# cxjyxxme/deep-online-video-stabilization

Hardware: AMD Instinct MI355X
Metric: stabilized frames/sec (720p, before_ch=31) (higher is better)
Workload: dtype f32 (bf16x3 split MFMA, f32 accumulate); 1 GPU; BASELINE.json configs[1]: v2_93 net, 1280x720, 1 stream(s)/GPU, batch=1 per stream, 13-ch stack from a 32-deep ring (lags 1,2,4,8,16,32; --before-ch 31 ignored as in the reference), ResNet-v2-50 regressor + 4x4 multi-grid warp + feedback; one independent stream set per GPU (replicas only); height=720, width=1280, streams_per_gpu=1, refine=1, operand_mode=4, launches_per_frame=64, hip_graph=True

## Files before the change

deep-online-video-stabilization_amd/csrc/conv.h:

```cpp
#pragma once
#include "common.h"

struct ConvArgs {
    const float* x;
    const float* w;
    float* y;
    const float* bias;
    const float* in_scale;
    const float* in_shift;
    const float* residual;
    const float* out_scale;
    const float* out_shift;
    const float* out_floor;
    float* partial;
    int N, H, W, Cin, Ho, Wo, Cout, KH, KW, stride, pad;
    int up;
    int res_H, res_W, res_stride;
    int relu_out;
    int x_ld, res_ld;
    int M, K;
    int splitk, steps_per_split;
    int cin_real;
    unsigned div_hw_mul, div_hw_shift, div_w_mul, div_w_shift;
    int rowrun;
    int in_scale_expected;
    int xcd_swizzle;
};

size_t conv_plan(ConvArgs& a);
struct Prof;
int conv_launch(const ConvArgs& a, hipStream_t st, Prof* prof = nullptr, int bf16_operands = 0, const float* w_img = nullptr,
                bool lowk_ring = false);

enum ConvFamily {
    CONV_IGEMM,
    CONV_RING,
    CONV_RING_KG,
    CONV_RING_PRO,
    CONV_PACKED,
    CONV_PACKED_KG2,
    CONV_ASTAT
};
struct ConvRoute {
    int family;
    int tile, bk, nbuf;
    int mode;
    int operand;
    int kg, pro;
    int reduce;
    int prof_kind;
    int astat_bm;
};
ConvRoute conv_route(const ConvArgs& a, int operand_mode, bool has_image, bool bound, bool lowk_ring = false );
const char* conv_prof_kind_name(int kind);
size_t conv_weight_image_floats(int Cout, int K);
int launch_weight_split_image(const float* w, int Cout, int K, float* img, hipStream_t st);
struct WeightImageTable { long w_off[64], img_off[64], tprefix[65]; int Cout[64], K[64]; int n; };
void weight_image_table_add(WeightImageTable& t, long w_off, long img_off, int Cout, int K);
int launch_weight_split_images(const float* w_base, float* img_base, const WeightImageTable& t, hipStream_t st);
int conv_reduce_launches(const ConvArgs& a, int operand_mode = 0);

struct ConvPair { int m_tower, x_tower_floats ; long dx, dy, dres, dscale; };
bool conv_pair_supported(const ConvArgs& a);
int conv_launch_pair(const ConvArgs& a, const ConvPair& pr, hipStream_t st, Prof* prof = nullptr,
                     const float* w_img = nullptr );

bool conv_b2b_supported(const ConvArgs& c2, const ConvArgs& c3);
int conv_b2b_launch(const ConvArgs& c2, const ConvArgs& c3, hipStream_t st, Prof* prof = nullptr);

static inline void sn_fastdiv_make(unsigned d, unsigned& mul, unsigned& shift) {
    unsigned l = 0;
    while ((1ull << l) < d) ++l;
    mul = (unsigned)((((1ull << l) - d) << 32) / d + 1);
    shift = l;
}
#ifdef __HIPCC__
__device__ __forceinline__ int sn_fastdiv(int n, unsigned mul, unsigned shift) {
    return (int)((__umulhi(mul, (unsigned)n) + (unsigned)n) >> shift);
}
#endif
```

deep-online-video-stabilization_amd/csrc/conv.hip:

```cpp
#include "conv.h"
#include "prof.h"
#include <climits>
#include <cstdio>
#include <cstdlib>
#include <algorithm>
#include <string>
#include <vector>

#include "conv_kernel.h"
#include "conv_ring_kernel.h"
#include "conv_astat_kernel.h"
#include "conv_b2b_kernel.h"

template <int PAIR>
__device__ __forceinline__ void conv_splitk_reduce_body(const ConvArgs& p, const ConvPair& pr) {
    const size_t q = (size_t)blockIdx.x * 256 + threadIdx.x;
    const int c4n = p.Cout / 4;
    if (q >= (size_t)p.M * c4n) return;
    const int m = (int)(q / c4n);
    const int n = (int)(q - (size_t)m * c4n) * 4;
    const bool t1 = PAIR && m >= pr.m_tower;
    const size_t slab = (size_t)p.M * p.Cout;
    const float* src = p.partial + (size_t)m * p.Cout + n;
    float4 s = *reinterpret_cast<const float4*>(src);
    for (int z = 1; z < p.splitk; ++z) {
        const float4 t = *reinterpret_cast<const float4*>(src + z * slab);
        s.x += t.x; s.y += t.y; s.z += t.z; s.w += t.w;
    }
    if (p.bias != nullptr) {
        const float4 b = *reinterpret_cast<const float4*>(p.bias + n);
        s.x += b.x; s.y += b.y; s.z += b.z; s.w += b.w;
    }
    if (p.residual != nullptr) {
        size_t ri;
        if (p.res_stride == 1 && p.res_H == p.Ho && p.res_W == p.Wo) {
            ri = (size_t)m * p.res_ld + n;
        } else {
            const int img = sn_fastdiv(m, p.div_hw_mul, p.div_hw_shift);
            const int rr = m - img * (p.Ho * p.Wo);
            const int oy = sn_fastdiv(rr, p.div_w_mul, p.div_w_shift), ox = rr - oy * p.Wo;
            ri = (((size_t)img * p.res_H + oy * p.res_stride) * p.res_W + ox * p.res_stride) * p.res_ld + n;
        }
        const float4 t = *reinterpret_cast<const float4*>(p.residual + (t1 ? pr.dres : 0) + ri);
        s.x += t.x; s.y += t.y; s.z += t.z; s.w += t.w;
// ... 16 lines not shown
}
__global__ __launch_bounds__(256) void conv_splitk_reduce_pair_kernel(const ConvArgs p, const ConvPair pr) {
    conv_splitk_reduce_body<1>(p, pr);
}

enum TileId { T128x128 = 0, T128x64 = 1, T64x64 = 2 };

static void tile_dims(int t, int& bm, int& bn) {
    bm = (t == T64x64) ? 64 : 128;
    bn = (t == T128x128) ? 128 : 64;
}

static int env_int(const char* name, int dflt) {
    const char* v = getenv(name);
    return v ? atoi(v) : dflt;
}

struct ConvSwitches {
    int tile = env_int("STABNET_CONV_TILE", -1), splitk = env_int("STABNET_CONV_SPLITK", -1);
    int bk16 = env_int("STABNET_CONV_BK16", 0);
    int nbuf = env_int("STABNET_CONV_NBUF", 0);
    int tuning_table = env_int("STABNET_CONV_TUNING_TABLE", 1);
    int split_below = env_int("STABNET_CONV_SPLIT_BELOW", 400), split_target = env_int("STABNET_CONV_SPLIT_TARGET", 448);
    int xcd = env_int("STABNET_CONV_XCD", 1);
    int ring = env_int("STABNET_CONV_RING", 1), ring_wgs_per_cu = env_int("STABNET_CONV_RING_WGS_PER_CU", 3);
    int lowk_igemm = env_int("STABNET_CONV_LOWK_IGEMM", 1);
    int ring_pro = env_int("STABNET_CONV_RING_PRO", 1);
    int kgroups = env_int("STABNET_CONV_KGROUPS", 1), kgroups_pro = env_int("STABNET_CONV_KGROUPS_PRO", 1);
    int packed_kg2 = env_int("STABNET_CONV_PACKED_KG2", 1), packed_kg3 = env_int("STABNET_CONV_PACKED_KG3", 1);
    int packed_pro = env_int("STABNET_CONV_PACKED_PRO", 1);
    int packed_wgs_per_cu = env_int("STABNET_CONV_PACKED_WGS_PER_CU", 2);
    int astat = env_int("STABNET_CONV_ASTAT", 1), astat_min_m = env_int("STABNET_CONV_ASTAT_MIN_M", 0);
    int astat_min_cout = env_int("STABNET_CONV_ASTAT_MIN_COUT", 256);
    int b2b = env_int("STABNET_CONV_B2B", 1), b2b_wgs_per_cu = env_int("STABNET_CONV_B2B_WGS_PER_CU", 2);
};
static const ConvSwitches& sw() {
    static const ConvSwitches s;
    return s;
}

static int g_force_tile = -2, g_force_split = -1;
static int force_tile() { return g_force_tile == -2 ? sw().tile : g_force_tile; }
static int force_split() { return g_force_tile == -2 ? sw().splitk : g_force_split; }

static int conv_bk(const ConvArgs& a) { return (a.rowrun || (a.Cin % 32 == 0 && !sw().bk16)) ? 32 : 16; }
static int conv_total_steps(const ConvArgs& a) {
    if (a.rowrun) return a.KH * cdiv(a.KW * a.Cin, 32);
    return a.KH * a.KW * (a.Cin / conv_bk(a));
}

struct TuneEntry { int M, Cout, K, KH, ring, splitk; };
#include "conv_tuning_table.h"
#include "conv_tuning_table_packed.h"
static int g_tuning_profile = 0;
static std::vector<TuneEntry> g_tuning_runtime;

static int tuning_lookup(int M, int Cout, int K, int KH, int ring) {
    for (const TuneEntry& e : g_tuning_runtime)
        if (e.M == M && e.Cout == Cout && e.K == K && e.KH == KH && e.ring == ring) return e.splitk;
    if (sw().tuning_table && g_tuning_profile == 1)
        for (const TuneEntry& e : g_tuning_packed)
            if (e.M == M && e.Cout == Cout && e.K == K && e.KH == KH && e.ring == ring) return e.splitk;
    if (sw().tuning_table)
        for (const TuneEntry& e : g_tuning_builtin)
            if (e.M == M && e.Cout == Cout && e.K == K && e.KH == KH && e.ring == ring) return e.splitk;
    return 0;
// ... 43 lines not shown
    const int nbuf = sw().nbuf;
    bf16_out = (bm == 64 && bn == 64 && bk == 32) ? operand : 0;
    const bool one_stage = nbuf == 1 || (nbuf == 0 && mode == 0 && bm == 64 && bn == 64 && a.M >= 32768);
    nbuf_out = (bf16_out != 1 && one_stage) ? 1 : 2;
}

static bool ring_eligible(const ConvArgs& a, int tile, bool has_prologue, bool lowk_ring = false) {
    if (a.rowrun) return true;
    if (!lowk_ring && sw().lowk_igemm && a.KH == 1 && a.KW == 1 && a.Cin == 64 && a.x_ld == a.Cin && a.out_floor == nullptr) return false;
    return sw().ring && tile == T64x64 && !has_prologue && a.up == 1 && a.Cin % 32 == 0 && !sw().bk16;
}

static bool ring_pro_vectors_ok(const ConvArgs& a) {
    if (a.in_scale == nullptr || a.in_shift == nullptr) return true;
    const long d = (long)(a.in_shift - a.in_scale);
    return d >= 0 && d < (1L << 30);
}
static bool ring_pro_geometry(const ConvArgs& a, int operand, bool has_prologue) {
    return sw().ring_pro && sw().ring && operand != 1 && !sw().bk16 && has_prologue && a.KH == 1 && a.KW == 1 && a.stride == 1 && a.pad == 0 &&
           a.up == 1 && a.Cin % 32 == 0 && !a.rowrun && a.x_ld == a.Cin;
}
static bool ring_pro_eligible(const ConvArgs& a, int operand) {
    return ring_pro_geometry(a, operand, a.in_scale != nullptr) && a.out_scale == nullptr && a.out_floor == nullptr && ring_pro_vectors_ok(a);
}

static int conv_kgroups(const ConvArgs& a, int operand, bool ring, bool has_prologue) {
    if (!sw().kgroups || a.splitk < 2 || operand == 1) return 1;
    if (a.steps_per_split * a.splitk != conv_total_steps(a)) return 1;
    if (ring && a.splitk == 3 && !a.rowrun) return 3;
    if (sw().kgroups_pro && !ring && a.splitk == 2 && ring_pro_geometry(a, operand, has_prologue) && ring_pro_vectors_ok(a)) return 2;
    return 1;
}

static int route_prof_kind(const ConvRoute& r) {
    switch (r.family) {
        case CONV_IGEMM:
            return PK_KERNEL_CONV_BASE + r.mode * 6 + r.tile * 2 + (r.bk == 32 ? 1 : 0) + (r.nbuf == 1 ? 18 : 0) + 36 * r.operand;
        case CONV_PACKED: return PK_KERNEL_CONV_PACKED + (r.pro ? 3 : r.mode);
        case CONV_PACKED_KG2: return PK_KERNEL_CONV_PACKED + (r.pro ? 6 : 4 + r.mode);
        case CONV_ASTAT: return PK_KERNEL_CONV_ASTAT;
        default: break;
    }
    const int split = r.operand >= 2 ? PK_KERNEL_CONV_SPLIT + 8 * (r.operand - 2) : 0;
    if (r.family == CONV_RING) return split ? split + r.mode : PK_KERNEL_CONV_RING + r.mode + (r.operand ? 3 : 0);
    if (r.family == CONV_RING_PRO) return split ? split + 5 : PK_KERNEL_CONV_KG + 2;
    if (r.kg == 2) return split ? split + 6 : PK_KERNEL_CONV_KG + 3;
    return split ? split + 3 + r.mode : PK_KERNEL_CONV_KG + r.mode;
}

ConvRoute conv_route(const ConvArgs& a, int operand_mode, bool has_image, bool bound, bool lowk_ring) {
    const ConvSwitches& s = sw();
    const bool image = operand_mode == 4 && has_image;
    const int op = operand_mode == 4 ? 0 : operand_mode;
    int splitk_unused = 1;
    const int t = pick_tile(a, splitk_unused);
    const bool t64 = t == T64x64, bk32 = conv_bk(a) == 32;
    const bool has_pro = bound ? a.in_scale != nullptr : a.in_scale_expected != 0;
    const bool ring = ring_eligible(a, t, has_pro, lowk_ring && image);
    const bool slabs = !bound || a.splitk == 1 || a.partial != nullptr;
    int kg = t64 ? conv_kgroups(a, op, ring, has_pro) : 1;
    if (image && s.packed_kg3 && ring && kg == 3 && a.K % 32 == 0 && slabs) kg = 1;
    const bool pro = kg == 1 && !ring && t64 && bk32 && (bound ? ring_pro_eligible(a, op) : ring_pro_geometry(a, op, has_pro));
    const bool packed_pro = image && s.packed_pro && !ring && t64 && bk32 && ring_pro_geometry(a, op, has_pro) &&
                            (!bound || a.out_floor == nullptr)  && ring_pro_vectors_ok(a) && slabs;
    if (packed_pro) kg = 1;
    const bool packed = (image && ring && kg == 1 && a.K % 32 == 0) || packed_pro;
    const bool packed_kg2 = packed && s.packed_kg2 && a.splitk == 2 && !a.rowrun && a.steps_per_split * 2 == conv_total_steps(a);
    if (packed_kg2) kg = 2;
    const int astat_min_m = s.astat_min_m > 0 ? s.astat_min_m : ((long)a.Cout * a.K >= 128 * 1024 ? 2048 : 8192);
    const bool astat = packed && !packed_pro && !packed_kg2 && kg == 1 && a.splitk == 1 && s.astat && !lowk_ring && !a.rowrun &&
                       a.KH == 1 && a.KW == 1 && a.stride == 1 && a.pad == 0 && a.up == 1 && a.K <= 256 && a.Cout >= s.astat_min_cout &&
                       a.M >= astat_min_m;

    ConvRoute r{};
    r.tile = t;
    r.bk = bk32 ? 32 : 16;
    r.mode = (a.up > 1 || a.rowrun) ? 2 : (a.pad == 0 ? 0 : 1);
    r.operand = op;
    r.kg = kg;
    r.reduce = (a.splitk > 1 && kg == 1) ? 1 : 0;
    if (astat) {
        r.family = CONV_ASTAT;
        r.operand = 4;
        r.astat_bm = 32;
    } else if (packed) {
        r.family = packed_kg2 ? CONV_PACKED_KG2 : CONV_PACKED;
        r.operand = 4;
        r.pro = packed_pro ? 1 : 0;
    } else if (pro) {
        r.family = CONV_RING_PRO;
        r.pro = 1;
    } else if (kg > 1) {
        r.family = CONV_RING_KG;
        r.pro = kg == 2 ? 1 : 0;
    } else if (ring) {
        r.family = CONV_RING;
    } else {
        int bm, bn;
        tile_dims(t, bm, bn);
        r.family = CONV_IGEMM;
        igemm_variant(a, bm, bn, r.bk, r.mode, op, r.nbuf, r.operand);
    }
    r.prof_kind = route_prof_kind(r);
    return r;
}

int conv_reduce_launches(const ConvArgs& a, int operand_mode) {
    return a.splitk < 2 ? 0 : conv_route(a, operand_mode, operand_mode == 4, false).reduce;
}

const char* conv_prof_kind_name(int kind) {
    static const std::vector<std::string> names = [] {
        std::vector<std::string> v(PK_KERNEL_CONV_BASE + 144);
        char buf[96];
        auto ring = [&](int family, int mode, int operand, int kg, int pro) {
            ConvRoute r{};
            r.family = family; r.mode = mode; r.operand = operand; r.kg = kg; r.pro = pro;
            snprintf(buf, sizeof(buf), "conv_ring_f32_kernel<%d, %d, %d, %d>", mode, operand, kg, pro);
            v[route_prof_kind(r)] = buf;
        };
        for (int operand = 0; operand < 4; ++operand) {
            for (int mode = 0; mode < 3; ++mode) ring(CONV_RING, mode, operand, 1, 0);
            if (operand == 1) continue;
            ring(CONV_RING_KG, 0, operand, 3, 0); ring(CONV_RING_KG, 1, operand, 3, 0);
            ring(CONV_RING_PRO, 0, operand, 1, 1); ring(CONV_RING_KG, 0, operand, 2, 1);
        }
        for (int mode = 0; mode < 3; ++mode) ring(CONV_PACKED, mode, 4, 1, 0);
        ring(CONV_PACKED, 0, 4, 1, 1);
        ring(CONV_PACKED_KG2, 0, 4, 2, 0); ring(CONV_PACKED_KG2, 1, 4, 2, 0); ring(CONV_PACKED_KG2, 0, 4, 2, 1);
        {
            ConvRoute r{};
            r.family = CONV_ASTAT; r.astat_bm = 32;
            snprintf(buf, sizeof(buf), "conv_astat_f32_kernel<%d>", r.astat_bm);
            v[route_prof_kind(r)] = buf;
        }
        for (int i = 0; i < 144; ++i) {
            ConvRoute r{};
            r.family = CONV_IGEMM;
            r.operand = i / 36; r.nbuf = 2 - i / 18 % 2; r.mode = i / 6 % 3; r.tile = i / 2 % 3; r.bk = (i & 1) ? 32 : 16;
            int bm, bn;
            tile_dims(r.tile, bm, bn);
            snprintf(buf, sizeof(buf), "conv_igemm_f32_kernel<%d, %d, %d, %d, %d, %d, %d, %d>", bm, bn, r.bk, bm / 2, bn / 2, r.mode, r.nbuf, r.operand);
            v[route_prof_kind(r)] = buf;
        }
        for (int i = 0; i < 4; ++i) {
            snprintf(buf, sizeof(buf), "conv_igemm_f32_pair_kernel<64, 64, %d, 32, 32, %d>", (i & 1) ? 32 : 16, i / 2);
            v[PK_KERNEL_CONV_PAIR + i] = buf;
        }
        v[PK_KERNEL_CONV_B2B] = "conv_b2b_f32_kernel<2>";
        v[PK_KERNEL_CONV_B2B + 1] = "conv_b2b_f32_kernel<4>";
        return v;
    }();
    return (kind >= 0 && kind < (int)names.size() && !names[kind].empty()) ? names[kind].c_str() : nullptr;
}

template <int BM, int BN, int BK, int WM, int WN, int MODE, int NBUF, int BF16 = 0>
static int launch_one_nb(const ConvArgs& a, hipStream_t st) {
    constexpr size_t lds_op = NBUF * (size_t)(BM + BN) * (BK + 4) * sizeof(float);
    constexpr size_t lds_epi = 4 * (size_t)SN_EPI_WAVE_BYTES;
    constexpr size_t lds = lds_op > lds_epi ? lds_op : lds_epi;
    static bool configured = false;
    auto kern = conv_igemm_f32_kernel<BM, BN, BK, WM, WN, MODE, NBUF, BF16>;
    if (!configured) {
        if (lds > 64 * 1024) {
            hipError_t e = hipFuncSetAttribute(reinterpret_cast<const void*>(kern),
                                               hipFuncAttributeMaxDynamicSharedMemorySize, (int)lds);
            if (e != hipSuccess) {
                stabnet_set_error("conv: hipFuncSetAttribute(%zu B LDS) failed: %s", lds, hipGetErrorString(e));
// ... 76 lines not shown
static int launch_ring_route(const ConvRoute& r, const ConvArgs& a, hipStream_t st) {
    int cus = 0;
    if (const int rc = device_cus(cus)) return rc;
    const int per_cu = r.kg > 1 ? 1 : (r.operand == 4 ? sw().packed_wgs_per_cu : sw().ring_wgs_per_cu);
    const long ntiles = (long)cdiv(a.M, 64) * cdiv(a.Cout, 64) * (r.kg > 1 ? 1 : a.splitk);
    const int grid = (int)std::min<long>(ntiles, (long)per_cu * usable_cus(cus));
    bool ok = false;
    switch (r.operand) {
        case 0: ok = launch_ring_operand<0>(r, a, grid, st); break;
        case 1: ok = launch_ring_operand<1>(r, a, grid, st); break;
        case 2: ok = launch_ring_operand<2>(r, a, grid, st); break;
        case 3: ok = launch_ring_operand<3>(r, a, grid, st); break;
        case 4: ok = launch_ring_operand<4>(r, a, grid, st); break;
        default: break;
    }
    SN_REQUIRE(ok, "conv: no conv_ring_f32_kernel<%d, %d, %d, %d>", r.mode, r.operand, r.kg, r.pro);
    SN_LAUNCH_CHECK("conv_ring_f32_kernel");
    return STABNET_OK;
}

static int launch_astat(const ConvRoute& r, const ConvArgs& a, hipStream_t st) {
    int cus = 0;
    if (const int rc = device_cus(cus)) return rc;
    const int bm = r.astat_bm;
    SN_REQUIRE(bm == 32 && a.K % 32 == 0 && (size_t)bm * a.K * 6 <= (size_t)SN_ASTAT_A_BYTES && a.splitk == 1,
               "conv: the A-stationary kernel takes BM %d x K %d without a K split only if the planes fit %d bytes", bm, a.K, SN_ASTAT_A_BYTES);
    const int mtiles = cdiv(a.M, bm), nblk = 2 * cdiv(a.Cout, 64);
    int groups = (int)std::min<long>(cdiv(nblk, 4), std::max<long>(1, 2L * usable_cus(cus) / mtiles));
    groups = cdiv(nblk, 4 * cdiv(cdiv(nblk, groups), 4));
    const dim3 grid(mtiles, groups);
    conv_astat_f32_kernel<32><<<grid, 256, 0, st>>>(a);
    SN_LAUNCH_CHECK("conv_astat_f32_kernel");
    return STABNET_OK;
}

size_t conv_weight_image_floats(int Cout, int K) { return (size_t)cdiv(Cout, 64) * (size_t)(K / 32) * 3072; }

__device__ __forceinline__ unsigned weight_split_head(float& x0, float& x1) {
    const float top = __builtin_bit_cast(float, 0x7F7F0000u), fmax = __builtin_bit_cast(float, 0x7F7FFFFFu);
    const float h0 = (fabsf(x0) > top && fabsf(x0) <= fmax) ? copysignf(top, x0) : x0;
    const float h1 = (fabsf(x1) > top && fabsf(x1) <= fmax) ? copysignf(top, x1) : x1;
    const unsigned p = sn_pack_bf16(h0, h1);
    x0 = sn_sub_f32(x0, __builtin_bit_cast(float, p << 16));
    x1 = sn_sub_f32(x1, __builtin_bit_cast(float, p & 0xffff0000u));
    return p;
}
__device__ __forceinline__ SnSplit3 weight_split3(const f32x4 x) {
    float a = x.x, b = x.y, c = x.z, d = x.w;
    typedef unsigned u32x2 __attribute__((ext_vector_type(2)));
    u32x2 h, m, l;
    h.x = weight_split_head(a, b); h.y = weight_split_head(c, d);
    m.x = sn_split_level(a, b); m.y = sn_split_level(c, d);
    l.x = sn_pack_bf16(a, b); l.y = sn_pack_bf16(c, d);
    SnSplit3 s;
    s.h = __builtin_bit_cast(sn_bf16x4, h); s.m = __builtin_bit_cast(sn_bf16x4, m); s.l = __builtin_bit_cast(sn_bf16x4, l);
    return s;
}

__device__ __forceinline__ void weight_split_image_thread(const float* __restrict__ w, int Cout, int K, uint4* __restrict__ img, long i) {
    const int steps = K / 32;
    const int lane = (int)(i & 63), j = (int)((i >> 6) & 1), wn = (int)((i >> 7) & 1);
    const long ts = i >> 8;
    const int ks = (int)(ts % steps), nt = (int)(ts / steps);
    const int n = nt * 64 + wn * 32 + (lane & 31), g = lane >> 5;
    f32x4 lo = {0.f, 0.f, 0.f, 0.f}, hi = lo;
    if (n < Cout) {
// ... 39 lines not shown

int launch_weight_split_image(const float* w, int Cout, int K, float* img, hipStream_t st) {
    SN_REQUIRE(w && img && Cout > 0 && K > 0 && K % 32 == 0, "weight image: K=%d must be a multiple of 32", K);
    const long total = (long)cdiv(Cout, 64) * (K / 32) * 256;
    weight_split_image_kernel<<<cdiv(total, 256), 256, 0, st>>>(w, Cout, K, reinterpret_cast<uint4*>(img));
    SN_LAUNCH_CHECK("weight_split_image_kernel");
    return STABNET_OK;
}

int conv_launch(const ConvArgs& a, hipStream_t st, Prof* prof, int bf16_operands, const float* w_img, bool lowk_ring) {
    SN_REQUIRE(a.rowrun || a.Cin % 16 == 0, "conv: Cin=%d must be a multiple of 16 (pad the channels)", a.Cin);
    SN_REQUIRE(!a.rowrun || (a.in_scale == nullptr && a.up == 1 && a.KH <= 8 && cdiv(a.KW * a.Cin, 32) <= 4),
               "conv: row-run operand needs no prologue, KH <= 8 and KW*Cin <= 128");
    SN_REQUIRE(a.Cout % 4 == 0, "conv: Cout=%d must be a multiple of 4", a.Cout);
    SN_REQUIRE(a.splitk >= 1 && a.steps_per_split >= 1 && a.div_hw_mul != 0, "conv: conv_plan() not called");
    SN_REQUIRE(a.splitk == 1 || a.partial != nullptr, "conv: split-K needs a workspace");
    const ConvRoute r = conv_route(a, bf16_operands, w_img != nullptr, true, lowk_ring);
    SN_REQUIRE(r.family != CONV_IGEMM || a.x_ld == a.Cin, "conv: a strided input (x_ld %d != Cin %d) needs the ring kernel", a.x_ld, a.Cin);
    const bool rec = prof != nullptr && prof->begin(st);
    int rc;
    switch (r.family) {
        case CONV_IGEMM: rc = launch_igemm(r, a, st); break;
        case CONV_PACKED:
        case CONV_PACKED_KG2: {
            ConvArgs b = a;
            b.w = w_img;
            rc = launch_ring_route(r, b, st);
            break;
        }
        case CONV_ASTAT: {
            ConvArgs b = a;
            b.w = w_img;
            rc = launch_astat(r, b, st);
            break;
        }
        default: rc = launch_ring_route(r, a, st); break;
    }
    if (rec) prof->end(st, r.prof_kind, 2.0 * a.M * (double)(a.KH * a.KW * (a.cin_real ? a.cin_real : a.Cin)) * a.Cout,
                       4.0 * ((double)a.N * a.H * a.W * a.Cin + (double)a.K * a.Cout + (double)a.M * a.Cout * (r.reduce ? a.splitk : 1) +
                              ((a.residual != nullptr && !r.reduce) ? (double)a.M * a.Cout : 0.0)),
                       a.M, a.Cout, a.K, a.splitk);
    if (rc) return rc;
    if (r.reduce) {
        const size_t q = (size_t)a.M * (a.Cout / 4);
        const bool rec2 = prof != nullptr && prof->begin(st);
        conv_splitk_reduce_kernel<<<cdiv((long)q, 256), 256, 0, st>>>(a);
        if (rec2) prof->end(st, PK_KERNEL_SPLITK_REDUCE, 0.0, 4.0 * (double)a.M * a.Cout * (a.splitk + 1 + (a.residual != nullptr ? 1 : 0)));
        SN_LAUNCH_CHECK("conv_splitk_reduce_kernel");
    }
    return STABNET_OK;
}

bool conv_pair_supported(const ConvArgs& a) {
    int splitk_unused = 1;
    const int t = pick_tile(a, splitk_unused);
    const bool pro = a.in_scale != nullptr || a.in_scale_expected;
    return t == T64x64 && !ring_eligible(a, t, pro) && a.up == 1 && !a.rowrun && (a.x_ld == 0 || a.x_ld == a.Cin);
}

template <int BK, int MODE>
static int launch_pair_one(const ConvArgs& a, const ConvPair& pr, hipStream_t st) {
    constexpr size_t lds = 2 * (size_t)(64 + 64) * (BK + 4) * sizeof(float);
    static_assert(lds >= 4 * (size_t)SN_EPI_WAVE_BYTES && lds <= 64 * 1024, "LDS of the 64x64 tile");
    dim3 grid(cdiv(a.M, 64), cdiv(a.Cout, 64), a.splitk);
    conv_igemm_f32_pair_kernel<64, 64, BK, 32, 32, MODE><<<grid, 256, lds, st>>>(a, pr);
    SN_LAUNCH_CHECK("conv_igemm_f32_pair_kernel");
// ... 148 lines not shown
                          int Cout, int KH, int KW, int stride, int pad, int relu_out, void* workspace,
                          size_t workspace_bytes, void* stream);

int stabnet_conv2d_fwd(const float* x, const float* w_ohwi, const float* bias, const float* in_scale,
                       const float* in_shift, const float* residual, int res_H, int res_W, int res_stride, float* y,
                       int N, int H, int W, int Cin, int Cout, int KH, int KW, int stride, int pad, int relu_out,
                       void* workspace, size_t workspace_bytes, void* stream) {
    return stabnet_conv2d_fwd_ex(x, w_ohwi, bias, in_scale, in_shift, residual, res_H, res_W, res_stride, nullptr, nullptr,
                                 y, N, H, W, Cin, Cout, KH, KW, stride, pad, relu_out, workspace, workspace_bytes, stream);
}

int stabnet_conv2d_fwd_ex(const float* x, const float* w_ohwi, const float* bias, const float* in_scale,
                          const float* in_shift, const float* residual, int res_H, int res_W, int res_stride,
                          const float* out_scale, const float* out_shift, float* y, int N, int H, int W, int Cin,
                          int Cout, int KH, int KW, int stride, int pad, int relu_out, void* workspace,
                          size_t workspace_bytes, void* stream) {
    SN_REQUIRE(x && w_ohwi && y, "conv2d_fwd: null pointer");
    SN_REQUIRE((out_scale == nullptr) == (out_shift == nullptr), "conv2d_fwd: out_scale and out_shift go together");
    ConvArgs a;
    int rc = fill_args(a, x, w_ohwi, bias, in_scale, in_shift, residual, res_H, res_W, res_stride, y, N, H, W, Cin, Cout,
                       KH, KW, stride, pad, relu_out);
    if (rc) return rc;
    const size_t need = conv_plan(a);
    if (need > workspace_bytes || (need > 0 && workspace == nullptr)) {
        stabnet_set_error("conv2d_fwd: workspace %zu B < %zu B needed", workspace_bytes, need);
        return STABNET_ERR_WORKSPACE;
    }
    a.partial = static_cast<float*>(workspace);
    a.out_scale = out_scale;
    a.out_shift = out_shift;
    return conv_launch(a, (hipStream_t)stream);
}

size_t stabnet_conv_weight_image_floats(int Cout, int KH, int KW, int Cin) {
    const int K = KH * KW * Cin;
    return (Cout > 0 && K > 0 && K % 32 == 0) ? conv_weight_image_floats(Cout, K) : 0;
}

int stabnet_conv_weight_split_image(const float* w_ohwi, int Cout, int KH, int KW, int Cin, float* w_img, void* stream) {
    SN_REQUIRE(w_ohwi && w_img, "conv_weight_split_image: null pointer");
    SN_REQUIRE(Cin % 32 == 0, "conv_weight_split_image: Cin=%d must be a multiple of 32", Cin);
    return launch_weight_split_image(w_ohwi, Cout, KH * KW * Cin, w_img, (hipStream_t)stream);
}

static size_t plan_packed(ConvArgs& a, int splitk) {
    size_t need = conv_plan(a);
    if (splitk > 0) {
        const int total = conv_total_steps(a);
        a.steps_per_split = cdiv(total, std::min(splitk, total));
        a.splitk = cdiv(total, a.steps_per_split);
        need = a.splitk > 1 ? (size_t)a.splitk * a.M * a.Cout * sizeof(float) : 0;
    }
    return need;
}

int stabnet_conv2d_packed_kind(int N, int H, int W, int Cin, int Cout, int KH, int KW, int stride, int pad, int prologue, int splitk) {
    ConvArgs a;
    if (fill_args(a, nullptr, nullptr, nullptr, nullptr, nullptr, nullptr, 0, 0, 1, nullptr, N, H, W, Cin, Cout, KH, KW, stride, pad, 0))
        return STABNET_ERR_BAD_ARG;
    a.in_scale_expected = prologue ? 1 : 0;
    (void)plan_packed(a, splitk);
    return conv_route(a, 4, true, false).prof_kind;
}

int stabnet_conv2d_fwd_packed(const float* x, const float* w_ohwi, const float* w_img, const float* bias, const float* in_scale,
                              const float* in_shift, const float* residual, int res_H, int res_W, int res_stride,
                              const float* out_scale, const float* out_shift, float* y, int N, int H, int W, int Cin,
                              int Cout, int KH, int KW, int stride, int pad, int relu_out, int splitk, void* workspace,
                              size_t workspace_bytes, void* stream) {
    SN_REQUIRE(x && w_ohwi && w_img && y, "conv2d_fwd_packed: null pointer");
    SN_REQUIRE((out_scale == nullptr) == (out_shift == nullptr), "conv2d_fwd_packed: out_scale and out_shift go together");
    ConvArgs a;
    int rc = fill_args(a, x, w_ohwi, bias, in_scale, in_shift, residual, res_H, res_W, res_stride, y, N, H, W, Cin, Cout,
                       KH, KW, stride, pad, relu_out);
    if (rc) return rc;
    const size_t need = plan_packed(a, splitk);
    if (need > workspace_bytes || (need > 0 && workspace == nullptr)) {
        stabnet_set_error("conv2d_fwd_packed: workspace %zu B < %zu B needed", workspace_bytes, need);
        return STABNET_ERR_WORKSPACE;
    }
    a.partial = static_cast<float*>(workspace);
    a.out_scale = out_scale;
    a.out_shift = out_shift;
    return conv_launch(a, (hipStream_t)stream, nullptr, 4, w_img);
}

int stabnet_conv3x3_conv1x1_fwd(const float* x, int x_ld, const float* w2_ohwi, const float* mid_scale, const float* mid_shift,
                                const float* w3_ohwi, const float* bias3, const float* residual, int res_H, int res_W,
                                int res_stride, int res_ld, const float* out_scale, const float* out_shift, float* y, int N, int H,
                                int W, int C, int Cout, int stride, int relu_out, void* stream) {
    SN_REQUIRE(x && w2_ohwi && mid_scale && mid_shift && w3_ohwi && y, "conv3x3_conv1x1_fwd: null pointer");
    SN_REQUIRE((out_scale == nullptr) == (out_shift == nullptr), "conv3x3_conv1x1_fwd: out_scale and out_shift go together");
    ConvArgs c2, c3;
    int rc = fill_args(c2, x, w2_ohwi, nullptr, nullptr, nullptr, nullptr, 0, 0, 1, nullptr, N, H, W, C, C, 3, 3, stride, 1, 1);
    if (rc) return rc;
    c2.x_ld = x_ld;
    (void)conv_plan(c2);
    c2.out_scale = mid_scale;
    c2.out_shift = mid_shift;
    rc = fill_args(c3, nullptr, w3_ohwi, bias3, nullptr, nullptr, residual, res_H, res_W, res_stride, y, N, c2.Ho, c2.Wo, C, Cout,
                   1, 1, 1, 0, relu_out);
    if (rc) return rc;
    c3.res_ld = res_ld;
    (void)conv_plan(c3);
    c3.out_scale = out_scale;
    c3.out_shift = out_shift;
    SN_REQUIRE(conv_b2b_supported(c2, c3), "conv3x3_conv1x1_fwd: C must be 64 or 128, Cout a multiple of C, stride 1 or 2");
    return conv_b2b_launch(c2, c3, (hipStream_t)stream);
// ... 4 lines not shown
```

deep-online-video-stabilization_amd/csrc/prof.h:

```cpp
#pragma once
#include <vector>
#include "common.h"

enum {
    PK_KERNEL_PAD = 1, PK_KERNEL_POOL = 2, PK_KERNEL_GAP = 3, PK_KERNEL_FC = 4, PK_KERNEL_MESH = 5,
    PK_KERNEL_WARP = 6, PK_KERNEL_ASSEMBLE = 7, PK_KERNEL_PUSH = 8, PK_KERNEL_SPLITK_REDUCE = 9, PK_KERNEL_WGRAD = 10, PK_KERNEL_HEAD = 20,
    PK_KERNEL_MJPEG_TRANSFORM = 30, PK_KERNEL_MJPEG_ENTROPY = 31, PK_KERNEL_MJPEG_LAYOUT = 32, PK_KERNEL_MJPEG_GATHER = 33 ,
    PK_KERNEL_INGEST_GREY_ROWS = 34, PK_KERNEL_INGEST_GREY_COLS = 35, PK_KERNEL_INGEST_COLOUR = 36 ,
    PK_KERNEL_MAP_SHRINK = 37, PK_KERNEL_REMAP_SRC = 38, PK_KERNEL_REMAP_SRC4 = 39 ,
    PK_KERNEL_REMAP_WIN = 60, PK_KERNEL_REMAP_WIN4 = 61 ,
    PK_KERNEL_REMAP_WIN_DEV = 62, PK_KERNEL_REMAP_WIN4_DEV = 63 ,
    PK_KERNEL_TF_GET_IMG = 64 ,
    PK_KERNEL_TVL1_STEP = 57, PK_KERNEL_TVL1_FUSED = 58 ,
    PK_KERNEL_TVL1_DOWN = 65, PK_KERNEL_TVL1_GRAD = 66, PK_KERNEL_TVL1_WARP = 67, PK_KERNEL_TVL1_UP = 68, PK_KERNEL_TVL1_MAP = 69 ,
    PK_KERNEL_WGRAD_SAME = 11 ,
    PK_KERNEL_CONV_PAIR = 80 , PK_KERNEL_CONV_KG = 84 , PK_KERNEL_CONV_RING = 90 ,
    PK_KERNEL_CONV_PACKED = 70 ,
    PK_KERNEL_CONV_ASTAT = 77 ,
    PK_KERNEL_CONV_B2B = 96 ,
    PK_KERNEL_CONV_SPLIT = 40 ,
    PK_KERNEL_CONV_BASE = 100
};

struct Prof {
    std::vector<hipEvent_t> ev;
    std::vector<int> kind;
    std::vector<double> flops, bytes;
    std::vector<int> shape;
    int cap = 0, n = 0;
    bool begin(hipStream_t st) {
        if (n >= cap) return false;
        (void)hipEventRecord(ev[2 * n], st);
        return true;
    }
    void end(hipStream_t st, int k, double f, double b, int sm = 0, int sn = 0, int sk = 0, int ss = 0) {
        (void)hipEventRecord(ev[2 * n + 1], st);
        kind[n] = k; flops[n] = f; bytes[n] = b;
        shape[4 * n] = sm; shape[4 * n + 1] = sn; shape[4 * n + 2] = sk; shape[4 * n + 3] = ss;
        ++n;
    }
};
```

include/stabnet_hip.h:

```cpp
#ifndef STABNET_HIP_H
#define STABNET_HIP_H

#include <stddef.h>
#include <stdint.h>

#ifdef __cplusplus
extern "C" {
#endif

const char* stabnet_last_error(void);
int stabnet_abi_version(void);


int stabnet_get_4_pts(const float* theta, int N, int grid_h, int grid_w, float do_crop_rate,
                      float* pts1, float* pts2, float* Hs, void* stream);

int stabnet_transformer_fwd(const float* pts2, const float* U, int N, int H, int W, int C, int grid_h, int grid_w,
                            float* out, float* black, float* x_map, float* y_map, float* Hs, void* stream);

int stabnet_warp_fwd(const float* theta, const float* U, int N, int H, int W, int C, int grid_h, int grid_w,
                     float do_crop_rate, float* out, float* black, float* x_map, float* y_map, float* Hs,
                     float* pts2, void* stream);

int stabnet_maps_from_hs_fwd(const float* Hs, const float* U, int N, int H, int W, int C, int grid_h, int grid_w,
                             float* out, float* black, float* x_map, float* y_map, void* stream);

int stabnet_interp_fwd(const float* im, const float* x, const float* y, int N, int H, int W, int C, float* out,
                       void* stream);


size_t stabnet_conv2d_workspace_bytes(int N, int H, int W, int Cin, int Cout, int KH, int KW, int stride, int pad);
void stabnet_conv_tuning_override(int tile, int splitk);
void stabnet_conv_tuning_table_set(int M, int Cout, int K, int KH, int ring, int splitk);
void stabnet_conv_tuning_profile(int profile);
int stabnet_conv2d_fwd(const float* x, const float* w_ohwi, const float* bias, const float* in_scale,
                       const float* in_shift, const float* residual, int res_H, int res_W, int res_stride, float* y,
                       int N, int H, int W, int Cin, int Cout, int KH, int KW, int stride, int pad, int relu_out,
                       void* workspace, size_t workspace_bytes, void* stream);
int stabnet_conv2d_fwd_ex(const float* x, const float* w_ohwi, const float* bias, const float* in_scale,
                          const float* in_shift, const float* residual, int res_H, int res_W, int res_stride,
                          const float* out_scale, const float* out_shift, float* y, int N, int H, int W, int Cin,
                          int Cout, int KH, int KW, int stride, int pad, int relu_out, void* workspace,
                          size_t workspace_bytes, void* stream);
size_t stabnet_conv_weight_image_floats(int Cout, int KH, int KW, int Cin);
int stabnet_conv_weight_split_image(const float* w_ohwi, int Cout, int KH, int KW, int Cin, float* w_img, void* stream);
int stabnet_conv2d_fwd_packed(const float* x, const float* w_ohwi, const float* w_img, const float* bias, const float* in_scale,
                              const float* in_shift, const float* residual, int res_H, int res_W, int res_stride,
                              const float* out_scale, const float* out_shift, float* y, int N, int H, int W, int Cin,
                              int Cout, int KH, int KW, int stride, int pad, int relu_out, int splitk, void* workspace,
                              size_t workspace_bytes, void* stream);
int stabnet_conv2d_packed_kind(int N, int H, int W, int Cin, int Cout, int KH, int KW, int stride, int pad, int prologue, int splitk);
int stabnet_conv3x3_conv1x1_fwd(const float* x, int x_ld, const float* w2_ohwi, const float* mid_scale, const float* mid_shift,
                                const float* w3_ohwi, const float* bias3, const float* residual, int res_H, int res_W,
                                int res_stride, int res_ld, const float* out_scale, const float* out_shift, float* y, int N, int H,
                                int W, int C, int Cout, int stride, int relu_out, void* stream);

int stabnet_net_create(void** net, int N, int H, int W, int in_ch, int n_theta, int keep_activations);
void stabnet_net_destroy(void* net);
int stabnet_net_set_bf16_operands(void* net, int on);
int stabnet_net_num_params(const void* net);
int stabnet_net_param_info(const void* net, int idx, char* name, int name_cap, long* offset, int* kind, int* dims4,
                           int* aux);
size_t stabnet_net_param_floats(const void* net);
size_t stabnet_net_trainable_floats(const void* net);
size_t stabnet_net_bn_channels(const void* net);
size_t stabnet_net_workspace_bytes(const void* net);
double stabnet_net_flops(const void* net);
int stabnet_net_num_launches(const void* net);
int stabnet_deploy_frame_launches(const void* net, int grid_h, int grid_w);
int stabnet_net_activation_info(const void* net, const char* name, long* offset, int* dims4);

int stabnet_net_fold_bn(const void* net, const float* params, float* fold, float eps, void* stream);
size_t stabnet_net_fold_floats(const void* net);

int stabnet_backbone_fwd_infer(const void* net, const float* params, const float* fold, const float* x_tensor,
                               float* theta, void* workspace, size_t workspace_bytes, void* stream, void* prof);


int stabnet_pad_channels(const float* x, float* y, long npix, int C, int Cp, void* stream);

int stabnet_stem_repack(const float* w, float* out, int Cout, int KH, int KW, int CinPad, int Cin, void* stream);

int stabnet_merge_vectors(const float* b_sc, const float* scale1, const float* shift1, int depth, int dbn, float* out, void* stream);
// ... 256 lines not shown
```

Baseline: 657.6 frames/s.

## Add patch-stationary 3x3 conv kernel holding bf16x3 input halo in LDS

```diff
diff --git a/deep-online-video-stabilization_amd/csrc/conv.h b/deep-online-video-stabilization_amd/csrc/conv.h
--- a/deep-online-video-stabilization_amd/csrc/conv.h
+++ b/deep-online-video-stabilization_amd/csrc/conv.h
@@ -39,7 +39,8 @@
     CONV_RING_PRO,
     CONV_PACKED,
     CONV_PACKED_KG2,
-    CONV_ASTAT
+    CONV_ASTAT,
+    CONV_PATCH
 };
 struct ConvRoute {
     int family;
@@ -50,6 +51,7 @@
     int reduce;
     int prof_kind;
     int astat_bm;
+    int patch_cfg;
 };
 ConvRoute conv_route(const ConvArgs& a, int operand_mode, bool has_image, bool bound, bool lowk_ring = false );
 const char* conv_prof_kind_name(int kind);
diff --git a/deep-online-video-stabilization_amd/csrc/conv.hip b/deep-online-video-stabilization_amd/csrc/conv.hip
--- a/deep-online-video-stabilization_amd/csrc/conv.hip
+++ b/deep-online-video-stabilization_amd/csrc/conv.hip
@@ -10,6 +10,7 @@
 #include "conv_kernel.h"
 #include "conv_ring_kernel.h"
 #include "conv_astat_kernel.h"
+#include "conv_patch_kernel.h"
 #include "conv_b2b_kernel.h"
 
 template <int PAIR>
@@ -92,6 +93,8 @@
     int packed_wgs_per_cu = env_int("STABNET_CONV_PACKED_WGS_PER_CU", 2);
     int astat = env_int("STABNET_CONV_ASTAT", 1), astat_min_m = env_int("STABNET_CONV_ASTAT_MIN_M", 0);
     int astat_min_cout = env_int("STABNET_CONV_ASTAT_MIN_COUT", 256);
+    int patch = env_int("STABNET_CONV_PATCH", 1), patch_min_m = env_int("STABNET_CONV_PATCH_MIN_M", 0);
+    int patch_cfg = env_int("STABNET_CONV_PATCH_CFG", 0);
     int b2b = env_int("STABNET_CONV_B2B", 1), b2b_wgs_per_cu = env_int("STABNET_CONV_B2B_WGS_PER_CU", 2);
 };
 static const ConvSwitches& sw() {
@@ -201,6 +204,18 @@
     return 1;
 }
 
+struct PatchForm { int ph, pw, wr, ns; };
+static const PatchForm g_patch_forms[] = {{8, 8, 1, 3}, {8, 8, 2, 3}};
+constexpr int SN_PATCH_FORMS = 2;
+constexpr size_t SN_PATCH_LDS_MAX = 160 * 1024;
+static int patch_cfg(const ConvArgs& a) {
+    auto fits = [&](int cfg) { return sn_patch_lds_bytes(g_patch_forms[cfg - 1].ph, g_patch_forms[cfg - 1].pw, a.Cin) <= SN_PATCH_LDS_MAX; };
+    const int forced = sw().patch_cfg;
+    if (forced >= 1 && forced <= SN_PATCH_FORMS) return fits(forced) ? forced : 0;
+    const int cfg = a.Cout <= 64 ? 1 : 2;
+    return fits(cfg) ? cfg : 0;
+}
+
 static int route_prof_kind(const ConvRoute& r) {
     switch (r.family) {
         case CONV_IGEMM:
@@ -208,6 +223,7 @@
         case CONV_PACKED: return PK_KERNEL_CONV_PACKED + (r.pro ? 3 : r.mode);
         case CONV_PACKED_KG2: return PK_KERNEL_CONV_PACKED + (r.pro ? 6 : 4 + r.mode);
         case CONV_ASTAT: return PK_KERNEL_CONV_ASTAT;
+        case CONV_PATCH: return PK_KERNEL_CONV_PATCH + r.patch_cfg - 1;
         default: break;
     }
     const int split = r.operand >= 2 ? PK_KERNEL_CONV_SPLIT + 8 * (r.operand - 2) : 0;
@@ -240,6 +256,10 @@
     const bool astat = packed && !packed_pro && !packed_kg2 && kg == 1 && a.splitk == 1 && s.astat && !lowk_ring && !a.rowrun &&
                        a.KH == 1 && a.KW == 1 && a.stride == 1 && a.pad == 0 && a.up == 1 && a.K <= 256 && a.Cout >= s.astat_min_cout &&
                        a.M >= astat_min_m;
+    const int patch_form = patch_cfg(a);
+    const bool patch = packed && !packed_pro && ((kg == 1 && a.splitk == 1) || packed_kg2) && s.patch && !lowk_ring && !a.rowrun &&
+                       a.KH == 3 && a.KW == 3 && a.stride == 1 && a.pad == 1 && a.up == 1 && a.Cin % 32 == 0 && patch_form != 0 &&
+                       a.M >= (s.patch_min_m > 0 ? s.patch_min_m : 12288);
 
     ConvRoute r{};
     r.tile = t;
@@ -252,6 +272,10 @@
         r.family = CONV_ASTAT;
         r.operand = 4;
         r.astat_bm = 32;
+    } else if (patch) {
+        r.family = CONV_PATCH;
+        r.operand = 4;
+        r.patch_cfg = patch_form;
     } else if (packed) {
         r.family = packed_kg2 ? CONV_PACKED_KG2 : CONV_PACKED;
         r.operand = 4;
@@ -303,6 +327,13 @@
             snprintf(buf, sizeof(buf), "conv_astat_f32_kernel<%d>", r.astat_bm);
             v[route_prof_kind(r)] = buf;
         }
+        for (int cfg = 1; cfg <= SN_PATCH_FORMS; ++cfg) {
+            ConvRoute r{};
+            r.family = CONV_PATCH; r.patch_cfg = cfg;
+            const PatchForm& f = g_patch_forms[cfg - 1];
+            snprintf(buf, sizeof(buf), "conv_patch_f32_kernel<%d, %d, %d, %d>", f.ph, f.pw, f.wr, f.ns);
+            v[route_prof_kind(r)] = buf;
+        }
         for (int i = 0; i < 144; ++i) {
             ConvRoute r{};
             r.family = CONV_IGEMM;
@@ -445,6 +476,41 @@
     conv_astat_f32_kernel<32><<<grid, 256, 0, st>>>(a);
     SN_LAUNCH_CHECK("conv_astat_f32_kernel");
     return STABNET_OK;
+}
+
+template <int PH, int PW, int WR, int NS>
+static int launch_patch_one(const ConvArgs& a, int cus, hipStream_t st) {
+    const size_t lds = sn_patch_lds_bytes(PH, PW, a.Cin);
+    auto kern = conv_patch_f32_kernel<PH, PW, WR, NS>;
+    static size_t configured = 64 * 1024;
+    if (lds > configured) {
+        hipError_t e = hipFuncSetAttribute(reinterpret_cast<const void*>(kern), hipFuncAttributeMaxDynamicSharedMemorySize, (int)SN_PATCH_LDS_MAX);
+        if (e != hipSuccess) {
+            stabnet_set_error("conv: hipFuncSetAttribute(%zu B LDS) failed: %s", SN_PATCH_LDS_MAX, hipGetErrorString(e));
+            return STABNET_ERR_LAUNCH;
+        }
+        configured = SN_PATCH_LDS_MAX;
+    }
+    constexpr int cs = 4 / ((PH / 4) * (PW / 8) / WR);
+    const int mtiles = a.N * cdiv(a.Ho, PH) * cdiv(a.Wo, PW), nblk = 2 * cdiv(a.Cout, 64);
+    const long slots = (long)std::min<size_t>(WR >= 4 ? 1 : 2, SN_PATCH_LDS_MAX / lds) * usable_cus(cus);
+    int groups = (int)std::min<long>(cdiv(nblk, cs), std::max<long>(1, slots / mtiles));
+    groups = cdiv(nblk, cs * cdiv(cdiv(nblk, groups), cs));
+    const dim3 grid(mtiles, groups);
+    kern<<<grid, 256, lds, st>>>(a);
+    SN_LAUNCH_CHECK("conv_patch_f32_kernel");
+    return STABNET_OK;
+}
+static int launch_patch(const ConvRoute& r, const ConvArgs& a, hipStream_t st) {
+    int cus = 0;
+    if (const int rc = device_cus(cus)) return rc;
+    SN_REQUIRE(a.KH == 3 && a.KW == 3 && a.stride == 1 && a.pad == 1 && a.up == 1 && a.Cin % 32 == 0 &&
+                   (a.splitk == 1 || (a.splitk == 2 && a.steps_per_split * 2 == conv_total_steps(a))) && a.Ho == a.H && a.Wo == a.W && r.patch_cfg >= 1 &&
+                   r.patch_cfg <= SN_PATCH_FORMS &&
+                   sn_patch_lds_bytes(g_patch_forms[r.patch_cfg - 1].ph, g_patch_forms[r.patch_cfg - 1].pw, a.Cin) <= SN_PATCH_LDS_MAX,
+               "conv: the patch-stationary kernel takes 3x3 / pad 1 / stride 1 over Cin %d (a multiple of 32) without a K split or with two equal K halves only if the planes fit %zu bytes",
+               a.Cin, SN_PATCH_LDS_MAX);
+    return r.patch_cfg == 1 ? launch_patch_one<8, 8, 1, 3>(a, cus, st) : launch_patch_one<8, 8, 2, 3>(a, cus, st);
 }
 
 size_t conv_weight_image_floats(int Cout, int K) { return (size_t)cdiv(Cout, 64) * (size_t)(K / 32) * 3072; }
@@ -550,6 +616,12 @@
             ConvArgs b = a;
             b.w = w_img;
             rc = launch_astat(r, b, st);
+            break;
+        }
+        case CONV_PATCH: {
+            ConvArgs b = a;
+            b.w = w_img;
+            rc = launch_patch(r, b, st);
             break;
         }
         default: rc = launch_ring_route(r, a, st); break;
@@ -764,6 +836,11 @@
     return conv_launch(a, (hipStream_t)stream);
 }
 
+int stabnet_conv2d_fwd_packed_ld(const float* x, int x_ld, const float* w_ohwi, const float* w_img, const float* bias, const float* in_scale,
+                                 const float* in_shift, const float* residual, int res_H, int res_W, int res_stride,
+                                 const float* out_scale, const float* out_shift, float* y, int N, int H, int W, int Cin,
+                                 int Cout, int KH, int KW, int stride, int pad, int relu_out, int splitk, void* workspace,
+                                 size_t workspace_bytes, void* stream);
 size_t stabnet_conv_weight_image_floats(int Cout, int KH, int KW, int Cin) {
     const int K = KH * KW * Cin;
     return (Cout > 0 && K > 0 && K % 32 == 0) ? conv_weight_image_floats(Cout, K) : 0;
@@ -800,12 +877,23 @@
                               const float* out_scale, const float* out_shift, float* y, int N, int H, int W, int Cin,
                               int Cout, int KH, int KW, int stride, int pad, int relu_out, int splitk, void* workspace,
                               size_t workspace_bytes, void* stream) {
+    return stabnet_conv2d_fwd_packed_ld(x, 0, w_ohwi, w_img, bias, in_scale, in_shift, residual, res_H, res_W, res_stride, out_scale, out_shift,
+                                        y, N, H, W, Cin, Cout, KH, KW, stride, pad, relu_out, splitk, workspace, workspace_bytes, stream);
+}
+
+int stabnet_conv2d_fwd_packed_ld(const float* x, int x_ld, const float* w_ohwi, const float* w_img, const float* bias, const float* in_scale,
+                                 const float* in_shift, const float* residual, int res_H, int res_W, int res_stride,
+                                 const float* out_scale, const float* out_shift, float* y, int N, int H, int W, int Cin,
+                                 int Cout, int KH, int KW, int stride, int pad, int relu_out, int splitk, void* workspace,
+                                 size_t workspace_bytes, void* stream) {
     SN_REQUIRE(x && w_ohwi && w_img && y, "conv2d_fwd_packed: null pointer");
     SN_REQUIRE((out_scale == nullptr) == (out_shift == nullptr), "conv2d_fwd_packed: out_scale and out_shift go together");
+    SN_REQUIRE(x_ld == 0 || (x_ld >= Cin && x_ld % 4 == 0), "conv2d_fwd_packed: x_ld=%d must be 0 or a multiple of 4 >= Cin=%d", x_ld, Cin);
     ConvArgs a;
     int rc = fill_args(a, x, w_ohwi, bias, in_scale, in_shift, residual, res_H, res_W, res_stride, y, N, H, W, Cin, Cout,
                        KH, KW, stride, pad, relu_out);
     if (rc) return rc;
+    a.x_ld = x_ld;
     const size_t need = plan_packed(a, splitk);
     if (need > workspace_bytes || (need > 0 && workspace == nullptr)) {
         stabnet_set_error("conv2d_fwd_packed: workspace %zu B < %zu B needed", workspace_bytes, need);
diff --git a/deep-online-video-stabilization_amd/csrc/conv_patch_kernel.h b/deep-online-video-stabilization_amd/csrc/conv_patch_kernel.h
--- /dev/null
+++ b/deep-online-video-stabilization_amd/csrc/conv_patch_kernel.h
@@ -0,0 +1,243 @@
+#pragma once
+#include "conv_kernel.h"
+
+#ifndef PATCH_ABLATE
+#define PATCH_ABLATE 0
+#endif
+
+constexpr int sn_patch_pixel_bytes(int cin) { return cin * 6 + 16; }
+constexpr int sn_patch_row_bytes(int pw, int cin) { return (((pw + 2) * sn_patch_pixel_bytes(cin) + 127) & ~255) + 128; }
+constexpr size_t sn_patch_lds_bytes(int ph, int pw, int cin) { return (size_t)(ph + 2) * sn_patch_row_bytes(pw, cin) + 4 * 4096; }
+
+template <int TM>
+__device__ __forceinline__ void conv_patch_epilogue(f32x16 (&acc)[TM][1], const ConvArgs& p, const int (&mrow)[TM][4], int m_safe, int nw0,
+                                                    int lane, float* scratch) {
+    const bool has_res = p.residual != nullptr;
+    const bool has_obn = p.out_scale != nullptr;
+    const bool has_bias = p.bias != nullptr;
+    const bool relu = p.relu_out;
+    const bool res_plain = p.res_stride == 1 && p.res_H == p.Ho && p.res_W == p.Wo;
+    float* const wr = scratch + (4 * (lane >> 5)) * 32 + (lane & 31);
+    const int rrow = lane >> 3, rc4 = (lane & 7) * 4;
+    const float* const rd = scratch + rrow * 32 + rc4;
+#pragma unroll
+    for (int i = 0; i < TM; ++i) {
+        unsigned roff[4];
+#pragma unroll
+        for (int q = 0; q < 4; ++q) {
+            const int m = mrow[i][q] >= 0 ? mrow[i][q] : m_safe;
+            if (!has_res || res_plain) {
+                roff[q] = (unsigned)(m * p.res_ld);
+            } else {
+                const int img = sn_fastdiv(m, p.div_hw_mul, p.div_hw_shift);
+                const int rr = m - img * (p.Ho * p.Wo);
+                const int oy = sn_fastdiv(rr, p.div_w_mul, p.div_w_shift), ox = rr - oy * p.Wo;
+                roff[q] = (unsigned)(((img * p.res_H + oy * p.res_stride) * p.res_W + ox * p.res_stride) * p.res_ld);
+            }
+        }
+        const int n = nw0 + rc4;
+        const bool ncol = n < p.Cout;
+        const int nc = min(n, p.Cout - 4);
+        float4 rv[4];
+        if (has_res) {
+#pragma unroll
+            for (int q = 0; q < 4; ++q) rv[q] = *reinterpret_cast<const float4*>(p.residual + (roff[q] + (unsigned)nc));
+        }
+        const float4 zero4 = make_float4(0.f, 0.f, 0.f, 0.f);
+        const float4 bv = has_bias ? *reinterpret_cast<const float4*>(p.bias + nc) : zero4;
+        const float4 os = has_obn ? *reinterpret_cast<const float4*>(p.out_scale + nc) : zero4;
+        const float4 ob = has_obn ? *reinterpret_cast<const float4*>(p.out_shift + nc) : zero4;
+        const bool has_floor = has_obn && p.out_floor != nullptr;
+        const float4 fl = has_floor ? *reinterpret_cast<const float4*>(p.out_floor + nc) : zero4;
+#pragma unroll
+        for (int r = 0; r < 16; ++r) wr[((r & 3) + 8 * (r >> 2)) * 32] = acc[i][0][r];
+        f32x4 t[4];
+#pragma unroll
+        for (int q = 0; q < 4; ++q) t[q] = *reinterpret_cast<const f32x4*>(rd + q * 256);
+#pragma unroll
+        for (int q = 0; q < 4; ++q) {
+            float4 v = make_float4(t[q].x, t[q].y, t[q].z, t[q].w);
+            v.x += bv.x; v.y += bv.y; v.z += bv.z; v.w += bv.w;
+            if (has_res) { v.x += rv[q].x; v.y += rv[q].y; v.z += rv[q].z; v.w += rv[q].w; }
+            if (has_obn) {
+                v.x = __builtin_fmaf(v.x, os.x, ob.x); v.y = __builtin_fmaf(v.y, os.y, ob.y);
+                v.z = __builtin_fmaf(v.z, os.z, ob.z); v.w = __builtin_fmaf(v.w, os.w, ob.w);
+            }
+            if (has_floor) { v.x = fmaxf(v.x, fl.x); v.y = fmaxf(v.y, fl.y); v.z = fmaxf(v.z, fl.z); v.w = fmaxf(v.w, fl.w); }
+            else if (relu) { v.x = fmaxf(v.x, 0.f); v.y = fmaxf(v.y, 0.f); v.z = fmaxf(v.z, 0.f); v.w = fmaxf(v.w, 0.f); }
+            if ((PATCH_ABLATE & 4) ? v.x == 123.456f : true)
+            if (ncol && mrow[i][q] >= 0) *reinterpret_cast<float4*>(p.y + ((size_t)mrow[i][q] * p.Cout + n)) = v;
+        }
+    }
+}
+
+template <int PH, int PW , int WR ,
+          int NS >
+__global__ __launch_bounds__(256, WR >= 4 ? 1 : 2) void conv_patch_f32_kernel(const ConvArgs p) {
+    constexpr int HW = PW + 2, NPIX = (PH + 2) * HW, RBX = PW / 8, RB = (PH / 4) * RBX;
+    static_assert(PH % 4 == 0 && PW % 8 == 0 && RB % WR == 0 && (RB / WR == 1 || RB / WR == 2) && NS >= 3, "row blocks of 4 x 8 pixels, one or two row units");
+    constexpr int RU = RB / WR;
+    constexpr int CS = 4 / RU;
+    typedef unsigned u32x2 __attribute__((ext_vector_type(2)));
+    extern __shared__ __attribute__((aligned(16))) unsigned char patch_lds[];
+
+    const int tid = threadIdx.x, lane = tid & 63, wave = __builtin_amdgcn_readfirstlane(tid >> 6);
+    const int csteps = p.Cin >> 5, steps = 9 * csteps;
+    const int PB = sn_patch_pixel_bytes(p.Cin), RPB = sn_patch_row_bytes(PW, p.Cin);
+    const ConvTile tile = conv_tile_of_block(p);
+    const int tiles_x = (p.Wo + PW - 1) / PW, tiles_img = tiles_x * ((p.Ho + PH - 1) / PH);
+    const int img = tile.mt / tiles_img, t_in = tile.mt - img * tiles_img;
+    const int oy0 = (t_in / tiles_x) * PH, ox0 = (t_in % tiles_x) * PW;
+    const int grp = tile.nt;
+
+    {
+        const int sub = tid & 7;
+        const unsigned ent = (unsigned)((sub >> 2) * 96 + (sub & 1) * 16 + ((sub >> 1) & 1) * 8);
+        const int nitems = NPIX * csteps;
+        constexpr int U = NPIX > 150 ? 8 : 4;
+        for (int it0 = tid >> 3; it0 < nitems; it0 += 32 * U) {
+            f32x4 v[U];
+            unsigned dst[U];
+            bool in[U];
+#pragma unroll
+            for (int i = 0; i < U; ++i) {
+                const int it = min(it0 + 32 * i, nitems - 1);
+                const int hp = it / csteps, cs = it - hp * csteps;
+                const int hy = hp / HW, hx = hp - hy * HW;
+                const int iy = oy0 - 1 + hy, ix = ox0 - 1 + hx;
+                in[i] = iy >= 0 && iy < p.H && ix >= 0 && ix < p.W;
+                const int iyc = min(max(iy, 0), p.H - 1), ixc = min(max(ix, 0), p.W - 1);
+                if (!(PATCH_ABLATE & 1)) v[i] = *reinterpret_cast<const f32x4*>(p.x + (size_t)((img * p.H + iyc) * p.W + ixc) * p.x_ld + (cs * 32 + sub * 4));
+                else v[i] = f32x4{(float)iyc, (float)ixc, (float)sub, 1.f};
+                dst[i] = (unsigned)(hy * RPB + hx * PB + cs * 192) + ent;
+            }
+            __builtin_amdgcn_sched_barrier(0);
+#pragma unroll
+            for (int i = 0; i < U; ++i) {
+                float a = in[i] ? v[i].x : 0.f, b = in[i] ? v[i].y : 0.f, c = in[i] ? v[i].z : 0.f, d = in[i] ? v[i].w : 0.f;
+                u32x2 h, m, l;
+                h.x = sn_split_level(a, b); h.y = sn_split_level(c, d);
+                m.x = sn_split_level(a, b); m.y = sn_split_level(c, d);
+                l.x = sn_pack_bf16(a, b); l.y = sn_pack_bf16(c, d);
+                *reinterpret_cast<u32x2*>(patch_lds + dst[i]) = h;
+                *reinterpret_cast<u32x2*>(patch_lds + dst[i] + 32) = m;
+                *reinterpret_cast<u32x2*>(patch_lds + dst[i] + 64) = l;
+            }
+        }
+    }
+    __syncthreads();
+
+    const int nblk = 2 * ((p.Cout + 63) >> 6);
+    const int bpg = (((nblk + (int)gridDim.y - 1) / (int)gridDim.y) + CS - 1) / CS * CS;
+    const int b_end = min(min(nblk, (grp + 1) * bpg), (p.Cout + 31) >> 5);
+    const int ru = wave % RU;
+    int b = grp * bpg + wave / RU;
+    if (b >= b_end) return;
+    float* const scratch = reinterpret_cast<float*>(patch_lds + (PH + 2) * RPB + wave * SN_EPI_WAVE_BYTES);
+    int mrow[WR][4];
+    unsigned blk_off[WR];
+#pragma unroll
+    for (int i = 0; i < WR; ++i) {
+        const int by = (ru * WR + i) / RBX, bx = (ru * WR + i) % RBX;
+        blk_off[i] = (unsigned)(4 * by * RPB + 8 * bx * PB);
+#pragma unroll
+        for (int q = 0; q < 4; ++q) {
+            const int oy = oy0 + 4 * by + q, ox = ox0 + 8 * bx + (lane >> 3);
+            mrow[i][q] = (oy < p.Ho && ox < p.Wo) ? (img * p.Ho + oy) * p.Wo + ox : -1;
+        }
+    }
+    const int m_safe = (img * p.Ho + oy0) * p.Wo + ox0;
+    const f32x4* lp = reinterpret_cast<const f32x4*>(p.w) + ((size_t)(b >> 1) * steps * 12 + (b & 1) * 6) * 64 + lane;
+    const unsigned char* const abase = patch_lds + (unsigned)(((lane & 31) >> 3) * RPB + (lane & 7) * PB + (lane >> 5) * 16);
+    const int items = ((b_end - b + CS - 1) / CS) * steps;
+    const int adv_block = 768 * ((CS / 2 - 1) * steps + 1);
+    int l_item = 0, l_ks = 0;
+    auto load = [&](f32x4 (&dst)[6]) {
+        if ((PATCH_ABLATE & 2) && l_item >= NS - 1) return;
+#pragma unroll
+        for (int i = 0; i < 6; ++i) dst[i] = lp[i * 64];
+        const int adv = l_item + 1 >= items ? 0 : (l_ks + 1 < steps ? 768 : adv_block);
+        lp += adv;
+        ++l_item;
+        l_ks = l_ks + 1 < steps ? l_ks + 1 : 0;
+        __builtin_amdgcn_sched_barrier(0);
+    };
+    f32x16 acc[WR][1], first_half[WR];
+    const int half = p.splitk == 2 ? steps >> 1 : steps;
+#pragma unroll
+    for (int i = 0; i < WR; ++i)
+#pragma unroll
+        for (int e = 0; e < 16; ++e) first_half[i][e] = 0.f;
+    auto zero = [&]() {
+#pragma unroll
+        for (int i = 0; i < WR; ++i)
+#pragma unroll
+            for (int e = 0; e < 16; ++e) acc[i][0][e] = 0.f;
+    };
+    int ks = 0, cs = 0, kw = 0;
+    unsigned a_off = 0;
+    auto item = [&](const f32x4 (&B)[6]) {
+#pragma unroll
+        for (int j = 0; j < 2; ++j) {
+            SnPlanes A[WR];
+#pragma unroll
+            for (int i = 0; i < WR; ++i) {
+                const unsigned char* ap = abase + (a_off + (unsigned)(j * 96) + blk_off[i]);
+                if (!(PATCH_ABLATE & 8)) {
+                    A[i].h = *reinterpret_cast<const sn_u32x4*>(ap);
+                    A[i].m = *reinterpret_cast<const sn_u32x4*>(ap + 32);
+                    A[i].l = *reinterpret_cast<const sn_u32x4*>(ap + 64);
+                } else {
+                    A[i].h = A[i].m = A[i].l = sn_u32x4{(unsigned)(size_t)ap, a_off, (unsigned)lane, 1u};
+                }
+            }
+            const sn_bf16x8 bh = __builtin_bit_cast(sn_bf16x8, B[j]), bm = __builtin_bit_cast(sn_bf16x8, B[2 + j]), bl = __builtin_bit_cast(sn_bf16x8, B[4 + j]);
+#define SN_PATCH_MFMA(ap_, b_)                                                                                                      \
+    _Pragma("unroll") for (int i = 0; i < WR; ++i)                                                                                  \
+        acc[i][0] = __builtin_amdgcn_mfma_f32_32x32x16_bf16(__builtin_bit_cast(sn_bf16x8, A[i].ap_), b_, acc[i][0], 0, 0, 0)
+            SN_PATCH_MFMA(l, bh);
+            SN_PATCH_MFMA(h, bl);
+            SN_PATCH_MFMA(m, bm);
+            SN_PATCH_MFMA(m, bh);
+            SN_PATCH_MFMA(h, bm);
+            SN_PATCH_MFMA(h, bh);
+#undef SN_PATCH_MFMA
+        }
+        a_off += 192;
+        if (++cs == csteps) {
+            cs = 0;
+            a_off += 16;
+            if (++kw == 3) { kw = 0; a_off += (unsigned)(RPB - 3 * PB); }
+        }
+        if (++ks == half && half != steps) {
+#pragma unroll
+            for (int i = 0; i < WR; ++i) first_half[i] = acc[i][0];
+            zero();
+        }
+        if (ks == steps) {
+            if (half != steps) {
+#pragma unroll
+                for (int i = 0; i < WR; ++i)
+#pragma unroll
+                    for (int e = 0; e < 16; ++e) acc[i][0][e] = first_half[i][e] + acc[i][0][e];
+            }
+            conv_patch_epilogue<WR>(acc, p, mrow, m_safe, b * 32, lane, scratch);
+            b += CS;
+            ks = 0;
+            a_off = 0;
+            zero();
+        }
+    };
+    f32x4 B[NS][6];
+    zero();
+#pragma unroll
+    for (int s = 0; s < NS - 1; ++s) load(B[s]);
+    for (int it = 0; it < items; it += NS) {
+#pragma unroll
+        for (int s = 0; s < NS; ++s) {
+            if (it + s >= items) break;
+            load(B[(s + NS - 1) % NS]);
+            item(B[s]);
+        }
+    }
+}
diff --git a/deep-online-video-stabilization_amd/csrc/prof.h b/deep-online-video-stabilization_amd/csrc/prof.h
--- a/deep-online-video-stabilization_amd/csrc/prof.h
+++ b/deep-online-video-stabilization_amd/csrc/prof.h
@@ -17,6 +17,7 @@
     PK_KERNEL_CONV_PAIR = 80 , PK_KERNEL_CONV_KG = 84 , PK_KERNEL_CONV_RING = 90 ,
     PK_KERNEL_CONV_PACKED = 70 ,
     PK_KERNEL_CONV_ASTAT = 77 ,
+    PK_KERNEL_CONV_PATCH = 24 ,
     PK_KERNEL_CONV_B2B = 96 ,
     PK_KERNEL_CONV_SPLIT = 40 ,
     PK_KERNEL_CONV_BASE = 100
diff --git a/include/stabnet_hip.h b/include/stabnet_hip.h
--- a/include/stabnet_hip.h
+++ b/include/stabnet_hip.h
@@ -49,6 +49,11 @@
                               const float* out_scale, const float* out_shift, float* y, int N, int H, int W, int Cin,
                               int Cout, int KH, int KW, int stride, int pad, int relu_out, int splitk, void* workspace,
                               size_t workspace_bytes, void* stream);
+int stabnet_conv2d_fwd_packed_ld(const float* x, int x_ld, const float* w_ohwi, const float* w_img, const float* bias, const float* in_scale,
+                                 const float* in_shift, const float* residual, int res_H, int res_W, int res_stride,
+                                 const float* out_scale, const float* out_shift, float* y, int N, int H, int W, int Cin,
+                                 int Cout, int KH, int KW, int stride, int pad, int relu_out, int splitk, void* workspace,
+                                 size_t workspace_bytes, void* stream);
 int stabnet_conv2d_packed_kind(int N, int H, int W, int Cin, int Cout, int KH, int KW, int stride, int pad, int prologue, int splitk);
 int stabnet_conv3x3_conv1x1_fwd(const float* x, int x_ld, const float* w2_ohwi, const float* mid_scale, const float* mid_shift,
                                 const float* w3_ohwi, const float* bias3, const float* residual, int res_H, int res_W,
```

After: 664.3 frames/s, median of 6. 1.0% higher.
